# hir0shim/singleSpMV

Hardware: NVIDIA B200
Metric: SpMV GFLOP/s (higher is better)
Workload: dtype f64

## Files before the change

singlespmv_b200/csrc/chunk_stream.cu:

```cuda
#include <algorithm>
#include <climits>
#include <cstdlib>
#include <cstring>
#include <map>

#include "chunk_stream.cuh"

namespace b2 {

template <typename VT, typename XT, typename AT, int MAXL, int TH, bool ACC, bool DICT>
__global__ void __launch_bounds__(TH)
chunk_stream_kernel(const int *__restrict__ ptr, const int *__restrict__ idx, const int *__restrict__ meta,
                    const VT *__restrict__ val, const XT *__restrict__ x, XT *__restrict__ y, int rowBegin, int rowEnd,
                    int chunk0, int nChunks, int capI, int capV, int S, int acc_mode)
{
    constexpr int MI = CS_META_INTS(TH);
    extern __shared__ __align__(128) unsigned char cs_smem[];
    __shared__ __align__(8) uint64_t bar[CS_MAXSTAGES];
    __shared__ int sbaseI[CS_MAXSTAGES], sbaseV[CS_MAXSTAGES];
    int *sidx = reinterpret_cast<int *>(cs_smem);
    VT *sval = reinterpret_cast<VT *>(cs_smem + (size_t)S * capI * sizeof(int));
    const int tid = threadIdx.x;
    const uint64_t pol_stream = policy_evict_first(), pol_x = policy_evict_last();

    auto issue = [&](int s, long long g, int b, int e) {
        const int *srcI = idx + b;
        const VT *srcV = val + b;
        const int misI = (int)((reinterpret_cast<uintptr_t>(srcI) & 15) / sizeof(int));
        const int misV = (int)((reinterpret_cast<uintptr_t>(srcV) & 15) / sizeof(VT));
        const int n = e - b;
        const uint32_t bytesI = DICT ? (uint32_t)(MI * sizeof(int)) : n ? (uint32_t)(((n + misI) * (int)sizeof(int) + 15) & ~15) : 0u;
        const uint32_t bytesV = n ? (uint32_t)(((n + misV) * (int)sizeof(VT) + 15) & ~15) : 0u;
        sbaseI[s] = b - misI;
        sbaseV[s] = b - misV;
        mbar_expect_tx(&bar[s], bytesI + bytesV);
        if (DICT) tma_load_1d(sidx + (size_t)s * capI, meta + g * MI, bytesI, &bar[s], pol_stream);
        if (n) {
            if (!DICT) tma_load_1d(sidx + (size_t)s * capI, srcI - misI, bytesI, &bar[s], pol_stream);
            tma_load_1d(sval + (size_t)s * capV, srcV - misV, bytesV, &bar[s], pol_stream);
        }
    };
    auto lo_of = [&](long long g) { return (int)min((long long)rowEnd, max((long long)rowBegin, g * TH)); };

    if (tid == 0)
        for (int s = 0; s < S; s++) mbar_init(&bar[s], 1);
    __syncthreads();
    if (tid == 0) {
        for (int s = 0; s < S; s++) {
            const long long c = (long long)blockIdx.x + (long long)s * gridDim.x;
            if (c < nChunks) issue(s, chunk0 + c, ptr[lo_of(chunk0 + c)], ptr[lo_of(chunk0 + c + 1)]);
        }
    }
    long long g = (long long)chunk0 + blockIdx.x;
    int r = (int)min(g * TH + tid, (long long)0x7fffffff);
    bool valid = r >= rowBegin && r < rowEnd;
    int p = 0, q = 0;
    if (!DICT && valid) {
        p = ptr[r];
        q = ptr[r + 1];
    }
    int k = 0;
    for (long long c = blockIdx.x; c < nChunks; c += gridDim.x, k++) {
        const int s = k % S;
        const long long cIssue = c + (long long)S * gridDim.x, cNext = c + gridDim.x;
        int nb = 0, ne = 0, pn = 0, qn = 0;
        if (tid == 0 && cIssue < nChunks) {
            nb = ptr[lo_of(chunk0 + cIssue)];
            ne = ptr[lo_of(chunk0 + cIssue + 1)];
        }
        const long long rnl = (chunk0 + cNext) * TH + tid;
        const int rn = (int)min(rnl, (long long)0x7fffffff);
        const bool validn = cNext < nChunks && rn >= rowBegin && rn < rowEnd;
        if (!DICT && validn) {
            pn = ptr[rn];
            qn = ptr[rn + 1];
        }
        const AT y0 = (ACC && valid) ? (AT)y[r] : (AT)0;
        mbar_wait(&bar[s], (uint32_t)(k / S) & 1u);
        AT acc = (ACC && acc_mode == CS_CONTINUE) ? y0 : (AT)0;
        XT xs[MAXL];
        int len, vo;
        if (DICT) {
            const int *rec = sidx + (size_t)s * capI;
            const uint32_t mrow = reinterpret_cast<const uint16_t *>(rec + CS_DICT + TH / 32)[tid];
            const int lane = tid & 31, cnt = __popc(mrow);
            int inc = cnt;
#pragma unroll
            for (int o = 1; o < 32; o <<= 1) {
                const int t = __shfl_up_sync(0xffffffffu, inc, o);
                if (lane >= o) inc += t;
            }
            vo = s * capV + (rec[CS_DICT + (tid >> 5)] + inc - cnt - sbaseV[s]);
            uint32_t m = valid ? mrow : 0u;
            len = __popc(m);
#pragma unroll
            for (int j = 0; j < MAXL; j++)
                if (j < len) {
                    xs[j] = ld_x(x + (r + rec[__ffs(m) - 1]), pol_x);
                    m &= m - 1;
                }
        } else {
            const int io = s * capI + (p - sbaseI[s]);
            vo = s * capV + (p - sbaseV[s]);
            len = q - p;
#pragma unroll
            for (int j = 0; j < MAXL; j++)
                if (j < len) xs[j] = ld_x(x + sidx[io + j], pol_x);
        }
#pragma unroll
        for (int j = 0; j < MAXL; j++)
            if (j < len) acc = Arith<AT>::add(acc, Arith<AT>::mul((AT)sval[vo + j], (AT)xs[j]));
        if (valid) y[r] = (XT)((ACC && acc_mode == CS_ADD) ? Arith<AT>::add(y0, acc) : acc);
        __syncthreads();
        if (tid == 0 && cIssue < nChunks) issue(s, chunk0 + cIssue, nb, ne);
        r = rn; p = pn; q = qn; valid = validn;
    }
}

__global__ void chunk_cap_kernel(const int *__restrict__ ptr, int nRow, int th, int nChunks, int *__restrict__ out)
{
    const int c = blockIdx.x * blockDim.x + threadIdx.x;
    int n = 0;
    if (c < nChunks) n = ptr[(int)min((long long)nRow, ((long long)c + 1) * th)] - ptr[(long long)c * th];
#pragma unroll
    for (int o = 16; o > 0; o >>= 1) n = max(n, __shfl_xor_sync(0xffffffffu, n, o));
    if ((threadIdx.x & 31) == 0 && n > 0) atomicMax(out, n);
}

template <int TH>
__global__ void __launch_bounds__(TH)
chunk_dict_kernel(const int *__restrict__ ptr, const int *__restrict__ idx, int nRow, int *__restrict__ meta,
                  int *__restrict__ overflow)
{
    __shared__ int red[2][TH / 32];
    __shared__ int dict[CS_DICT];
    const int tid = threadIdx.x, lane = tid & 31, w = tid >> 5;
    const long long r = (long long)blockIdx.x * TH + tid;
    int b = 0, n = 0;
    if (r < nRow) {
        b = ptr[r];
        n = ptr[r + 1] - b;
    }
    int off[CS_MAXLEN];
#pragma unroll
    for (int j = 0; j < CS_MAXLEN; j++) off[j] = j < n ? idx[b + j] - (int)r : INT_MAX;
    int nd = 0;
    for (int cur = INT_MIN;;) {
        int mn = INT_MAX;
#pragma unroll
        for (int j = 0; j < CS_MAXLEN; j++)
            if (off[j] > cur) mn = min(mn, off[j]);
        mn = __reduce_min_sync(0xffffffffu, mn);
        if (lane == 0) red[nd & 1][w] = mn;
        __syncthreads();
        mn = INT_MAX;
#pragma unroll
        for (int i = 0; i < TH / 32; i++) mn = min(mn, red[nd & 1][i]);
        if (mn == INT_MAX) break;
        if (nd == CS_DICT) {
            if (tid == 0) *overflow = 1;
            return;
        }
        if (tid == 0) dict[nd] = mn;
        cur = mn;
        nd++;
    }
    uint32_t m = 0;
    int last = -1;
    bool bad = false;
#pragma unroll
    for (int j = 0; j < CS_MAXLEN; j++)
        if (j < n) {
            int k = 0;
            for (int i = 0; i < nd; i++) k += dict[i] < off[j];
            bad |= k <= last;
            last = k;
            m |= 1u << k;
        }
    if (bad) *overflow = 1;
    int *rec = meta + (size_t)blockIdx.x * CS_META_INTS(TH);
    if (tid < CS_DICT) rec[tid] = tid < nd ? dict[tid] : 0;
    if (lane == 0) rec[CS_DICT + w] = ptr[min(r, (long long)nRow)];
    reinterpret_cast<uint16_t *>(rec + CS_DICT + TH / 32)[tid] = (uint16_t)m;
}

int ChunkStream::build(const int *ptr_d, const int *idx_d, const void *val_d, bool val_is_f32, int nRow_, int nnz,
                       int maxLen_, cudaStream_t s)
{
    ptr = ptr_d; idx = idx_d; val = val_d; f32 = val_is_f32; nRow = nRow_; maxLen = maxLen_;
    feed = CS_FEED_IDX;
    meta.release();
    static const int env_max = getenv("B200SPMV_TMA_MAXLEN") ? atoi(getenv("B200SPMV_TMA_MAXLEN")) : CS_MAXLEN;
    const int env_th = getenv("B200SPMV_TMA_R") ? atoi(getenv("B200SPMV_TMA_R")) : 0;
    ok = nnz > 0 && nRow > 0 && maxLen > 0 && maxLen <= std::min(env_max, CS_MAXLEN);
    if (!ok) return B200SPMV_OK;
    th = env_th == 512 ? 512 : 256;
    const int nChunks = ceil_div(nRow, th);
    const char *env_feed = getenv("B200SPMV_CS_FEED");
    const bool want_dict = !(env_feed && !strcmp(env_feed, "idx"));
    DevBuf<int> m;
    B2_TRY(m.alloc(2));
    B2_CUDA(cudaMemsetAsync(m.p, 0, 2 * sizeof(int), s));
    chunk_cap_kernel<<<ceil_div(nChunks, 256), 256, 0, s>>>(ptr, nRow, th, nChunks, m.p);
    B2_KERNEL_CHECK();
    const size_t metaInts = (size_t)nChunks * CS_META_INTS(th);
    if (want_dict) {
        B2_TRY(meta.alloc(metaInts + CS_SLACK));
        B2_CUDA(cudaMemsetAsync(meta.p + metaInts, 0, CS_SLACK * sizeof(int), s));
        if (th == 512) chunk_dict_kernel<512><<<nChunks, 512, 0, s>>>(ptr, idx, nRow, meta.p, m.p + 1);
        else chunk_dict_kernel<256><<<nChunks, 256, 0, s>>>(ptr, idx, nRow, meta.p, m.p + 1);
        B2_KERNEL_CHECK();
    }
    int h[2] = {0, 0};
    B2_CUDA(cudaMemcpyAsync(h, m.p, sizeof h, cudaMemcpyDeviceToHost, s));
    B2_CUDA(cudaStreamSynchronize(s));
    cap = h[0];
    if (want_dict && !h[1]) feed = CS_FEED_DICT;
    else meta.release();
    const size_t stage = (size_t)(cap + 16) * (f32 ? 4 : 8) + (feed == CS_FEED_DICT ? CS_META_INTS(th) * 4 : (size_t)(cap + 16) * 4);
    if (2 * stage > 200 * 1024) ok = false;
    return B200SPMV_OK;
}

template <typename VT, typename XT, typename AT, int MAXL, int TH, bool ACC, bool DICT>
static int cs_launch(const ChunkStream &c, const XT *x, XT *y, int rb, int re, int acc, cudaStream_t s)
{
    constexpr int VA = 16 / (int)sizeof(VT);
    static const int env_s = getenv("B200SPMV_TMA_S") ? atoi(getenv("B200SPMV_TMA_S")) : 0;
    static const int env_b = getenv("B200SPMV_TMA_CTAS") ? atoi(getenv("B200SPMV_TMA_CTAS")) : 0;
    const int S = (env_s >= 1 && env_s <= CS_MAXSTAGES) ? env_s : 2;
    const int capI = DICT ? CS_META_INTS(TH) : (c.cap + 8) & ~3, capV = (c.cap + 2 * VA) & ~(VA - 1);
    const size_t smem = (size_t)S * ((size_t)capI * 4 + (size_t)capV * sizeof(VT));
    auto kern = chunk_stream_kernel<VT, XT, AT, MAXL, TH, ACC, DICT>;
    static int sms = 0;
    static std::map<std::pair<int, size_t>, int> per_sm;
    int dev = 0;
    B2_CUDA(cudaGetDevice(&dev));
    if (!sms) B2_CUDA(cudaDeviceGetAttribute(&sms, cudaDevAttrMultiProcessorCount, dev));
    const auto key = std::make_pair(dev, smem);
    auto it = per_sm.find(key);
    if (it == per_sm.end()) {
        B2_CUDA(cudaFuncSetAttribute(kern, cudaFuncAttributeMaxDynamicSharedMemorySize, (int)std::max<size_t>(smem, 200 * 1024)));
        int n = 0;
        B2_CUDA(cudaOccupancyMaxActiveBlocksPerMultiprocessor(&n, kern, TH, smem));
        if (n < 1) { set_error("row-chunk stream: %zu bytes of shared memory do not fit", smem); return B200SPMV_ERR_UNSUPPORTED; }
        it = per_sm.emplace(key, n).first;
    }
    const int perSm = env_b > 0 ? std::min(it->second, env_b) : it->second;
    const int chunk0 = rb / TH, nChunks = ceil_div(re, TH) - chunk0;
    const int grid = std::min(nChunks, sms * perSm);
    kern<<<grid, TH, smem, s>>>(c.ptr, c.idx, c.meta.p, static_cast<const VT *>(c.val), x, y, rb, re, chunk0, nChunks, capI, capV, S, acc);
    B2_KERNEL_CHECK();
    return B200SPMV_OK;
}

template <typename VT, typename XT, typename AT, int MAXL, int TH, bool ACC>
static int cs_feed(const ChunkStream &c, const XT *x, XT *y, int rb, int re, int acc, cudaStream_t s)
{
    if (c.feed == CS_FEED_DICT) return cs_launch<VT, XT, AT, MAXL, TH, ACC, true>(c, x, y, rb, re, acc, s);
    return cs_launch<VT, XT, AT, MAXL, TH, ACC, false>(c, x, y, rb, re, acc, s);
}

template <typename VT, typename XT, typename AT>
static int cs_dispatch(const ChunkStream &c, const XT *x, XT *y, int rb, int re, int acc, cudaStream_t s)
{
#define CS_GO(MAXL)                                                                                       \
    do {                                                                                                  \
        if (c.th == 512 && acc) return cs_feed<VT, XT, AT, MAXL, 512, true>(c, x, y, rb, re, acc, s);   \
        if (c.th == 512) return cs_feed<VT, XT, AT, MAXL, 512, false>(c, x, y, rb, re, acc, s);         \
        if (acc) return cs_feed<VT, XT, AT, MAXL, 256, true>(c, x, y, rb, re, acc, s);                  \
        return cs_feed<VT, XT, AT, MAXL, 256, false>(c, x, y, rb, re, acc, s);                          \
    } while (0)
    if (c.maxLen <= 8) CS_GO(8);
    else CS_GO(16);
#undef CS_GO
}

int ChunkStream::run(const double *x, double *y, int rb, int re, int acc, cudaStream_t s) const
{
    if (rb < 0 || re > nRow || rb > re) { set_error("multiply_rows: bad row range [%d,%d) for %d rows", rb, re, nRow); return B200SPMV_ERR_INVALID; }
    if (rb == re) return B200SPMV_OK;
    if (f32) return cs_dispatch<float, double, double>(*this, x, y, rb, re, acc, s);
    return cs_dispatch<double, double, double>(*this, x, y, rb, re, acc, s);
}

int ChunkStream::run_f32(const float *x, float *y, int rb, int re, int acc, bool acc64, cudaStream_t s) const
{
    if (rb < 0 || re > nRow || rb > re) { set_error("multiply_rows: bad row range [%d,%d) for %d rows", rb, re, nRow); return B200SPMV_ERR_INVALID; }
    if (!f32) { set_error("row-chunk stream: fp32 vectors need fp32 value storage"); return B200SPMV_ERR_STATE; }
    if (rb == re) return B200SPMV_OK;
    if (acc64) return cs_dispatch<float, float, double>(*this, x, y, rb, re, acc, s);
    return cs_dispatch<float, float, float>(*this, x, y, rb, re, acc, s);
}

}
```

singlespmv_b200/csrc/chunk_stream.cuh:

```cuda
#pragma once
#include "common.cuh"

namespace b2 {

constexpr int CS_MAXLEN = 16;
constexpr int CS_SLACK = 8;
constexpr int CS_MAXSTAGES = 4;

constexpr int CS_DICT = 16;
__host__ __device__ constexpr int CS_META_INTS(int th) { return CS_DICT + th / 32 + th / 2; }
enum { CS_FEED_IDX = 0, CS_FEED_DICT = 1 };

struct ChunkStream {
    const int *ptr = nullptr, *idx = nullptr;
    const void *val = nullptr;
    bool f32 = false, ok = false;
    int nRow = 0, maxLen = 0, th = 0, cap = 0;
    int feed = CS_FEED_IDX;
    DevBuf<int> meta;

    int build(const int *ptr_d, const int *idx_d, const void *val_d, bool val_is_f32, int nRow_, int nnz, int maxLen_,
              cudaStream_t s);
    int run(const double *x, double *y, int rb, int re, int acc, cudaStream_t s) const;
    int run_f32(const float *x, float *y, int rb, int re, int acc, bool acc64, cudaStream_t s) const;
};

}
```

singlespmv_b200/csrc/crs.cu:

```cuda
#include <algorithm>
#include <cstdlib>
#include <cstring>

#include "chunk_stream.cuh"
#include "entry_stream.cuh"
#include "tile_stream.cuh"

namespace b2 {

__global__ void crs_to_f32_kernel(const double *__restrict__ in, int n, float *__restrict__ out)
{
    const int i = blockIdx.x * blockDim.x + threadIdx.x;
    if (i < n) out[i] = __double2float_rn(in[i]);
}
__global__ void crs_to_f64_kernel(const float *__restrict__ in, int n, double *__restrict__ out)
{
    const int i = blockIdx.x * blockDim.x + threadIdx.x;
    if (i < n) out[i] = (double)in[i];
}

constexpr int RBS_MAXLEN = 16;
constexpr int RBS_WARPS = 8;
constexpr int RBS_ITERS = 8;

// ... 81 lines not shown
    EntryStream es;
    bool use_es = false;
    int path_opt;
    int prec;
    explicit CrsFormat(const b200spmv_options &o) : f32(o.value_f32 != 0 || o.precision != 0), path_opt(o.crs_path), prec(o.precision) {}

    int convert(const CooView &A, cudaStream_t s) override
    {
        nRow = A.nRow; nCol = A.nCol; nnz = A.nnz;
        B2_TRY(validate_sorted_coo(A, s));
        B2_TRY(ptr.alloc((size_t)nRow + 1));
        B2_TRY(idx.alloc((size_t)nnz + CS_SLACK));
        B2_TRY(build_row_ptr(A.row, nnz, nRow, ptr.p, s));
        B2_CUDA(cudaMemcpyAsync(idx.p, A.col, sizeof(int) * (size_t)nnz, cudaMemcpyDeviceToDevice, s));
        if (f32) {
            val.release();
            B2_TRY(val32.alloc((size_t)nnz + CS_SLACK));
            if (nnz) crs_to_f32_kernel<<<ceil_div(nnz, 256), 256, 0, s>>>(A.val, nnz, val32.p);
            B2_KERNEL_CHECK();
            B2_TRY(ts.build(ptr.p, idx.p, val32.p, true, nRow, nnz, s));
        } else {
            B2_TRY(val.alloc((size_t)nnz + CS_SLACK));
            B2_CUDA(cudaMemcpyAsync(val.p, A.val, sizeof(double) * (size_t)nnz, cudaMemcpyDeviceToDevice, s));
            B2_TRY(ts.build(ptr.p, idx.p, val.p, false, nRow, nnz, s));
        }
        B2_TRY(max_row_length(ptr.p, nRow, &maxLen, s));
        B2_TRY(cs.build(ptr.p, idx.p, f32 ? (const void *)val32.p : (const void *)val.p, f32, nRow, nnz, maxLen, s));
        use_rbs = path_opt == 2 && !prec && rowblock_applies(maxLen, nnz);
        int band = 0;
        if (path_opt == 0 || path_opt == 4) B2_TRY(max_band(A.row, A.col, nnz, A.rowOffset, &band, s));
        short_rows = path_opt != 1 && path_opt != 4 && (use_rbs || (cs.ok && !gathers_need_l2(band)));
        static const char *force = getenv("B200SPMV_CRS_PATH");
        use_es = false;
        const bool force_es = force && !strcmp(force, "es") && path_opt == 0;
        if (!short_rows && !f32 && !prec && (path_opt == 4 || force_es || (path_opt == 0 && gathers_need_l2(band))) && !(force && !strcmp(force, "tile"))) {
            B2_TRY(es.build(ptr.p, idx.p, val.p, nRow, nnz, gathers_need_l2(band), s));
            use_es = es.ok;
        }
        B2_CUDA(cudaStreamSynchronize(s));
        return B200SPMV_OK;
    }

    int multiply(const double *x, double *y, cudaStream_t s) override { return multiply_rows(0, nRow, x, y, s); }
    int multiply_f32(const float *x, float *y, cudaStream_t s) override
    {
        if (!prec) { set_error("multiply_f32: the handle was created with precision = 0 (fp64 vectors)"); return B200SPMV_ERR_STATE; }
        if (short_rows && !use_rbs) return cs.run_f32(x, y, 0, nRow, CS_OVERWRITE, prec == 2, s);
        return ts.run_rows_f32(x, y, CS_OVERWRITE, 0, nRow, prec == 2, s);
    }

    int multiply_rows(int rb, int re, const double *x, double *y, cudaStream_t s) override
    {
        if (prec) { set_error("multiply: the handle was created with precision = %d, use b200spmv_multiply_f32", prec); return B200SPMV_ERR_STATE; }
        if (!short_rows && use_es) return es.run_rows(x, y, rb, re, s);
        if (!short_rows) return ts.run_rows(x, y, CS_OVERWRITE, rb, re, s);
        if (rb < 0 || re > nRow || rb > re) { set_error("multiply_rows: bad row range [%d,%d)", rb, re); return B200SPMV_ERR_INVALID; }
        if (rb == re) return B200SPMV_OK;
        if (use_rbs) return rowblock_spmv(ptr.p, idx.p, f32 ? (const void *)val32.p : (const void *)val.p, f32, maxLen, rb, re, x, y, s);
        return cs.run(x, y, rb, re, CS_OVERWRITE, s);
    }
    bool has_rows() const override { return !prec; }
    int prepare_rows(int rb, int re) override { return short_rows ? B200SPMV_OK : use_es ? es.prepare(rb, re) : ts.prepare(rb, re); }
    int col_extent(int rb, int re, int *cmin, int *cmax) override
    {
        if (rb < 0 || re > nRow || rb > re) { set_error("col_extent: bad row range [%d,%d)", rb, re); return B200SPMV_ERR_INVALID; }
        int pb = 0, pe = 0;
        B2_CUDA(cudaMemcpy(&pb, ptr.p + rb, sizeof(int), cudaMemcpyDeviceToHost));
        B2_CUDA(cudaMemcpy(&pe, ptr.p + re, sizeof(int), cudaMemcpyDeviceToHost));
        if (pe <= pb) { *cmin = 0; *cmax = -1; return B200SPMV_OK; }
        return minmax_i32(idx.p, pb, pe, cmin, cmax);
    }

    bool scalar(const std::string &n, long long *out) override
    {
        if (n == "alg_bytes") {
            *out = (f32 ? 8LL : 12LL) * nnz + 4LL * (nRow + 1) + (prec ? 4LL : 8LL) * ((long long)nCol + nRow);
            return true;
        }
        if (n == "launches") { *out = short_rows ? 1 : use_es ? (es.nTiles > 1 ? 2 : 1) + (es.nEmpty ? 1 : 0) : (ts.nTiles > 1 ? 2 : 1); return true; }
        if (n == "crs_kernel") { *out = short_rows ? 1 : use_es ? (es.tma ? 2 : 3) : 0; return true; }
        if (n == "maxLength") { *out = maxLen; return true; }
        if (n == "short_row_path") { *out = short_rows ? 1 : 0; return true; }
        if (n == "chunk_feed") { *out = short_rows && !use_rbs ? cs.feed : CS_FEED_IDX; return true; }
        if (n == "nTiles") { *out = ts.nTiles; return true; }
        if (n == "value_f32") { *out = f32 ? 1 : 0; return true; }
        if (n == "precision") { *out = prec; return true; }
        return false;
    }

    long long array(const std::string &n, void *dst, long long cap) override
    {
        if (n == "ptr") return export_device(ptr.p, ptr.bytes(), dst, cap);
        if (n == "idx") return export_device(idx.p, sizeof(int) * (size_t)nnz, dst, cap);
        if (n == "val") {
            if (!f32) return export_device(val.p, sizeof(double) * (size_t)nnz, dst, cap);
            if (!dst) return (long long)(sizeof(double) * (size_t)nnz);
            DevBuf<double> w;
            if (w.alloc((size_t)nnz)) return B200SPMV_ERR_NOMEM;
            if (nnz) crs_to_f64_kernel<<<ceil_div(nnz, 256), 256>>>(val32.p, nnz, w.p);
            return export_device(w.p, w.bytes(), dst, cap);
        }
        return -1000;
    }
};

Format *make_crs(const b200spmv_options &o) { return new CrsFormat(o); }

}
```

singlespmv_b200/csrc/ss.cu:

```cuda
#include <algorithm>
#include <cstdlib>
#include <cstring>
#include <cub/cub.cuh>

#include "chunk_stream.cuh"
#include "colblocks.cuh"
#include "tile_stream.cuh"

namespace b2 {

__global__ void ss_slab_kernel(const int *__restrict__ row, const int *__restrict__ col, const double *__restrict__ val,
                               long long nnz, long long slots, int padRow, int *__restrict__ row2d,
                               int *__restrict__ col2d, double *__restrict__ val2d)
{
    const long long p = (long long)blockIdx.x * blockDim.x + threadIdx.x;
    if (p >= slots) return;
    const bool real = p < nnz;
    row2d[p] = real ? row[p] : padRow;
    col2d[p] = real ? col[p] : 0;
    val2d[p] = real ? val[p] : 0.0;
}

__global__ void chain_mixed_kernel(const int *__restrict__ row2d, long long slots, int W, int *__restrict__ mixed)
{
// ... 219 lines not shown
    {
        nRow = A.nRow; nCol = A.nCol; nnz = A.nnz;
        B2_TRY(validate_sorted_coo(A, s));
        H = nnz / W + (nnz % W != 0);
        const long long slots = (long long)H * W;
        B2_TRY(row_ptr.alloc((size_t)nRow + 1));
        B2_TRY(row2d.alloc((size_t)slots));
        B2_TRY(col2d.alloc((size_t)slots + CS_SLACK));
        B2_TRY(val2d.alloc((size_t)slots + CS_SLACK));
        B2_TRY(seg_index.alloc((size_t)H));
        B2_TRY(build_row_ptr(A.row, nnz, nRow, row_ptr.p, s));
        if (slots) {
            ss_slab_kernel<<<ceil_div(slots, 256), 256, 0, s>>>(A.row, A.col, A.val, nnz, slots, nRow, row2d.p, col2d.p, val2d.p);
            B2_KERNEL_CHECK();
        }
        B2_TRY(build_chain(row2d.p, H, W, seg_index.p, &nStep, counts, segs, s));
        B2_TRY(ts.build(row_ptr.p, col2d.p, val2d.p, false, nRow, nnz, s));
        B2_TRY(max_row_length(row_ptr.p, nRow, &maxLen, s));
        B2_TRY(cs.build(row_ptr.p, col2d.p, val2d.p, false, nRow, nnz, maxLen, s));
        use_rbs = path_opt == 2 && rowblock_applies(maxLen, nnz);
        int band = 0;
        if (path_opt == 0 && cs.ok) B2_TRY(max_band(A.row, A.col, nnz, A.rowOffset, &band, s));
        short_rows = path_opt != 1 && (use_rbs || (cs.ok && !gathers_need_l2(band)));
        cb.reset();
        if (!faithful) B2_TRY(make_col_block_engine(A, row_ptr.p, cbs_want, s, &cb));
        if (faithful) B2_TRY(val_buf.alloc((size_t)slots));
        B2_CUDA(cudaStreamSynchronize(s));
        return B200SPMV_OK;
    }

    int multiply(const double *x, double *y, cudaStream_t s) override
    {
        if (!faithful) return multiply_rows(0, nRow, x, y, s);
        if (nRow == 0) return B200SPMV_OK;
        const long long slots = (long long)H * W;
        B2_TRY(prof.mark(0, s));
        if (slots) {
            ss_mul_kernel<<<ceil_div(slots, 256), 256, 0, s>>>(col2d.p, val2d.p, x, slots, val_buf.p);
            B2_KERNEL_CHECK();
        }
        B2_TRY(prof.mark(1, s));
        B2_TRY(faithful_fold(segs, counts, W, val_buf.p, s));
        ss_gather_kernel<<<ceil_div(nRow, 256), 256, 0, s>>>(row_ptr.p, val_buf.p, nRow, W, 0, y);
        B2_KERNEL_CHECK();
        B2_TRY(prof.mark(2, s));
        return prof.finish();
    }

    bool has_rows() const override { return !faithful && !(cb != nullptr); }
    int prepare_rows(int rb, int re) override
    {
        if (faithful) return B200SPMV_OK;
        if (cb != nullptr) return cb->prepare(rb, re);
        return short_rows ? B200SPMV_OK : ts.prepare(rb, re);
    }
    int col_extent(int rb, int re, int *cmin, int *cmax) override
    {
        if (rb < 0 || re > nRow || rb > re) { set_error("col_extent: bad row range [%d,%d)", rb, re); return B200SPMV_ERR_INVALID; }
        int pb = 0, pe = 0;
        B2_CUDA(cudaMemcpy(&pb, row_ptr.p + rb, sizeof(int), cudaMemcpyDeviceToHost));
        B2_CUDA(cudaMemcpy(&pe, row_ptr.p + re, sizeof(int), cudaMemcpyDeviceToHost));
        if (pe <= pb) { *cmin = 0; *cmax = -1; return B200SPMV_OK; }
        return minmax_i32(col2d.p, pb, pe, cmin, cmax);
    }
    int multiply_rows(int rb, int re, const double *x, double *y, cudaStream_t s) override
    {
        if (faithful) return Format::multiply_rows(rb, re, x, y, s);
        if ((cb != nullptr)) return cb->run(x, y, rb, re, s);
        if (short_rows) {
            if (rb < 0 || re > nRow || rb > re) { set_error("multiply_rows: bad row range [%d,%d)", rb, re); return B200SPMV_ERR_INVALID; }
            if (use_rbs) return rowblock_spmv(row_ptr.p, col2d.p, val2d.p, false, maxLen, rb, re, x, y, s);
            return cs.run(x, y, rb, re, CS_OVERWRITE, s);
        }
        return ts.run_rows(x, y, CS_OVERWRITE, rb, re, s);
    }

    bool scalar(const std::string &n, long long *out) override
    {
        if (prof.scalar(n, out)) return true;
        if (n == "col_blocks") { *out = (cb != nullptr) ? cb->n_blocks() : 0; return true; }
        if (n == "col_block_engine") { *out = (cb == nullptr) ? 0 : (cb->name()[0] == 'e' ? 1 : 2); return true; }
        if (n == "short_row_path") { *out = short_rows ? 1 : 0; return true; }
        if (n == "chunk_feed") { *out = !faithful && cb == nullptr && short_rows && !use_rbs ? cs.feed : CS_FEED_IDX; return true; }
        if (n == "H") { *out = H; return true; }
        if (n == "nStep") { *out = nStep; return true; }
        if (n == "W") { *out = W; return true; }
        if (n == "alg_bytes") {
            *out = 12LL * nnz + 4LL * (nRow + 1) + 8LL * nCol + 8LL * nRow;
            return true;
        }
        if (n == "launches") {
            if (!faithful) { *out = (cb != nullptr) ? cb->n_blocks() : short_rows ? 1 : (ts.nTiles > 1 ? 2 : 1); return true; }
            int l = 2;
            for (int c : counts) l += c > 0;
            *out = l;
            return true;
        }
        return false;
    }

    long long array(const std::string &n, void *dst, long long cap) override
    {
        if (n == "row_ptr") return export_device(row_ptr.p, row_ptr.bytes(), dst, cap);
        if (n == "row_idx") return export_device(row2d.p, row2d.bytes(), dst, cap);
        if (n == "col_idx") return export_device(col2d.p, sizeof(int) * (size_t)H * W, dst, cap);
        if (n == "val") return export_device(val2d.p, sizeof(double) * (size_t)H * W, dst, cap);
        if (n == "segment_index") return export_device(seg_index.p, seg_index.bytes(), dst, cap);
        if (n == "sum_segs") return export_device(segs.p, segs.bytes(), dst, cap);
        if (n == "sum_segs_count") return export_host(counts.data(), counts.size() * sizeof(int), dst, cap);
        return -1000;
    }
};

Format *make_ss(const b200spmv_options &o) { return new SsFormat(o); }

constexpr int CSS_HIST = 1024;
__global__ void css_block_key_kernel(const int *__restrict__ col, int nnz, int B, int nBlock, int *__restrict__ key,
                                     int *__restrict__ id, int *__restrict__ blockNnz)
{
    __shared__ int hist[CSS_HIST];
    const bool local = nBlock <= CSS_HIST;
    if (local)
        for (int k = threadIdx.x; k < nBlock; k += blockDim.x) hist[k] = 0;
    __syncthreads();
    for (int i = blockIdx.x * blockDim.x + threadIdx.x; i < nnz; i += gridDim.x * blockDim.x) {
        const int b = col[i] / B;
        key[i] = b;
        id[i] = i;
        atomicAdd(local ? &hist[b] : &blockNnz[b], 1);
    }
    __syncthreads();
    if (local)
        for (int k = threadIdx.x; k < nBlock; k += blockDim.x)
            if (hist[k]) atomicAdd(&blockNnz[k], hist[k]);
}
__global__ void css_scatter_kernel(const int *__restrict__ row, const int *__restrict__ col, const double *__restrict__ val,
                                   const int *__restrict__ key_sorted, const int *__restrict__ id_sorted, int nnz,
                                   const long long *__restrict__ slabBase, const int *__restrict__ blockStart,
                                   int *__restrict__ row2d, int *__restrict__ col2d, double *__restrict__ val2d)
{
    const int k = blockIdx.x * blockDim.x + threadIdx.x;
    if (k >= nnz) return;
    const int b = key_sorted[k], i = id_sorted[k];
    const long long p = slabBase[b] + (k - blockStart[b]);
    row2d[p] = row[i];
    col2d[p] = col[i];
    val2d[p] = val[i];
}

__global__ void colblock_spread_kernel(const int *__restrict__ ptr, const int *__restrict__ col, int nRow, int B,
                                       unsigned long long *__restrict__ stats)
{
    const int r = blockIdx.x * blockDim.x + threadIdx.x;
    int touched = 0, nonEmpty = 0;
    if (r < nRow) {
        int last = -1;
        for (int j = ptr[r]; j < ptr[r + 1]; j++) {
            const int b = col[j] / B;
            touched += b != last;
            last = b;
        }
        nonEmpty = touched > 0;
    }
#pragma unroll
    for (int o = 16; o > 0; o >>= 1) {
        touched += __shfl_xor_sync(0xffffffffu, touched, o);
// ... 141 lines not shown
        if (!faithful) {
            if (ellb) return ellb->run(x, y, 0, nRow, s);
            for (int b = 0; b < nBlock; b++) B2_TRY(blocks[(size_t)b]->run(x, y, 0, nRow, gather_bound, b > 0 ? CS_ADD : CS_OVERWRITE, s));
            return B200SPMV_OK;
        }
        const long long slots = (long long)totalH * W;
        B2_TRY(prof.mark(0, s));
        if (slots) {
            ss_mul_kernel<<<ceil_div(slots, 256), 256, 0, s>>>(col2d.p, val2d.p, x, slots, val_buf.p);
            B2_KERNEL_CHECK();
        }
        B2_TRY(prof.mark(1, s));
        B2_CUDA(cudaMemsetAsync(y, 0, sizeof(double) * (size_t)nRow, s));
        for (int b = 0; b < nBlock; b++) {
            CssBlock &k = *blocks[(size_t)b];
            B2_TRY(faithful_fold(k.segs, k.counts, W, val_buf.p + k.base, s));
            ss_gather_kernel<<<ceil_div(nRow, 256), 256, 0, s>>>(row_ptr.p + (size_t)b * ((size_t)nRow + 1), val_buf.p + k.base,
                                                                nRow, W, 1, y);
            B2_KERNEL_CHECK();
        }
        B2_TRY(prof.mark(2, s));
        return prof.finish();
    }

    bool has_rows() const override { return !faithful; }
    int prepare_rows(int rb, int re) override
    {
        if (faithful || ellb || (rb == 0 && re == nRow)) return B200SPMV_OK;
        for (auto &k : blocks) if (!k->cs.ok || gather_bound) B2_TRY(k->ts.prepare(rb, re));
        return B200SPMV_OK;
    }
    int multiply_rows(int rb, int re, const double *x, double *y, cudaStream_t s) override
    {
        if (faithful) return Format::multiply_rows(rb, re, x, y, s);
        if (rb < 0 || re > nRow || rb > re) { set_error("multiply_rows: bad row range [%d,%d)", rb, re); return B200SPMV_ERR_INVALID; }
        if (rb == re) return B200SPMV_OK;
        if (nBlock == 0) {
            B2_CUDA(cudaMemsetAsync(y + rb, 0, sizeof(double) * (size_t)(re - rb), s));
            return B200SPMV_OK;
        }
        if (ellb) return ellb->run(x, y, rb, re, s);
        for (int b = 0; b < nBlock; b++) B2_TRY(blocks[(size_t)b]->run(x, y, rb, re, gather_bound, b > 0 ? CS_ADD : CS_OVERWRITE, s));
        return B200SPMV_OK;
    }
    int multiply_continue(int rb, int re, const double *x, double *y, cudaStream_t s)
    {
        bool first = true;
        for (auto &k : blocks) {
            if (k->cnt == 0 && !first) continue;
            if (k->cnt == 0) { B2_CUDA(cudaMemsetAsync(y + rb, 0, sizeof(double) * (size_t)(re - rb), s)); first = false; continue; }
            B2_TRY(k->run(x, y, rb, re, gather_bound, first ? CS_OVERWRITE : CS_CONTINUE, s));
            first = false;
        }
        return B200SPMV_OK;
    }

    int n_x_slices() const override { return faithful || nBlock < 1 ? 1 : nBlock; }
    void x_slice(int i, long long *c0, long long *c1) const override
    {
        if (faithful || nBlock < 1) { *c0 = 0; *c1 = nCol; return; }
        *c0 = (long long)i * B;
        *c1 = std::min<long long>(nCol, *c0 + B);
    }
    int multiply_rows_slice(int i, int rb, int re, const double *x, double *y, cudaStream_t s) override
    {
        if (faithful || nBlock < 1) return multiply_rows(rb, re, x, y, s);
        if (ellb) return ellb->run_block(i, x, y, rb, re, s);
        return blocks[(size_t)i]->run(x, y, rb, re, gather_bound, i > 0 ? CS_ADD : CS_OVERWRITE, s);
    }

    bool scalar(const std::string &n, long long *out) override
    {
        if (prof.scalar(n, out)) return true;
        if (n == "B") { *out = B; return true; }
        if (n == "col_block_engine") { *out = ellb ? 1 : (gather_bound ? 2 : 0); return true; }
        if (n == "nBlock") { *out = nBlock; return true; }
        if (n == "chunk_feed") {
            bool any = false, all = true;
            if (!faithful && !ellb && !gather_bound)
                for (auto &k : blocks) if (k->cs.ok) { any = true; all = all && k->cs.feed == CS_FEED_DICT; }
            *out = any && all ? CS_FEED_DICT : CS_FEED_IDX;
            return true;
        }
        if (n == "totalH") { *out = totalH; return true; }
        if (n == "W") { *out = W; return true; }
        if (n == "alg_bytes") {
            *out = 12LL * nnz + 4LL * nBlock * ((long long)nRow + 1) + 8LL * nCol + 8LL * nRow;
            return true;
        }
        if (n == "launches") {
            long long l = 0;
            if (!faithful && ellb) l = ellb->n_blocks();
            else if (!faithful) for (auto &k : blocks) l += k->cs.ok ? 1 : (k->ts.nTiles > 1 ? 2 : 1);
            else { l = 2; for (auto &k : blocks) { l += 1; for (int c : k->counts) l += c > 0; } }
            *out = l;
            return true;
        }
        return false;
    }

    long long array(const std::string &n, void *dst, long long cap) override
    {
        if (n == "row_ptr") return export_device(row_ptr.p, row_ptr.bytes(), dst, cap);
        if (n == "row_idx") return export_device(row2d.p, row2d.bytes(), dst, cap);
        if (n == "col_idx") return export_device(col2d.p, sizeof(int) * (size_t)totalH * W, dst, cap);
        if (n == "val") return export_device(val2d.p, sizeof(double) * (size_t)totalH * W, dst, cap);
        if (n == "segment_index") return export_device(seg_index.p, seg_index.bytes(), dst, cap);
        std::vector<int> h;
        if (n == "H") { for (auto &k : blocks) h.push_back(k->H); return export_host(h.data(), h.size() * sizeof(int), dst, cap); }
        if (n == "nStep") { for (auto &k : blocks) h.push_back(k->nStep); return export_host(h.data(), h.size() * sizeof(int), dst, cap); }
        if (n == "sum_segs_count") {
            for (auto &k : blocks) h.insert(h.end(), k->counts.begin(), k->counts.end());
            return export_host(h.data(), h.size() * sizeof(int), dst, cap);
        }
        if (n == "sum_segs") {
            size_t total = 0;
            for (auto &k : blocks) total += k->segs.n;
            if (!dst) return (long long)(total * sizeof(int));
            if (cap < (long long)(total * sizeof(int))) { set_error("get_array: destination too small"); return B200SPMV_ERR_INVALID; }
            size_t at = 0;
            for (auto &k : blocks) {
                if (k->segs.n && cudaMemcpy((int *)dst + at, k->segs.p, k->segs.bytes(), cudaMemcpyDeviceToHost) != cudaSuccess) {
                    set_error("get_array: cudaMemcpy D2H failed");
                    return B200SPMV_ERR_CUDA;
                }
                at += k->segs.n;
            }
            return (long long)(total * sizeof(int));
        }
        return -1000;
    }
};

Format *make_css(const b200spmv_options &o) { return new CssFormat(o); }

struct CrsColBlocks : ColBlockEngine {
    CssFormat css;
    explicit CrsColBlocks(const b200spmv_options &o) : css(o) { css.lean = true; css.input_checked = true; }
    int run(const double *x, double *y, int rb, int re, cudaStream_t s) override { return css.multiply_continue(rb, re, x, y, s); }
    int prepare(int rb, int re) override { return css.prepare_rows(rb, re); }
    int n_blocks() const override { return css.nBlock; }
    const char *name() const override { return "crs"; }
};
int make_col_block_engine(const CooView &A, const int *row_ptr, int want, cudaStream_t s, std::unique_ptr<ColBlockEngine> *out)
{
    out->reset();
    static const char *env_n = getenv("B200SPMV_COL_BLOCKS");
    if (env_n) want = atoi(env_n) == 0 ? -1 : atoi(env_n);
    if (want < 0 || A.nnz == 0 || A.nRow == 0 || A.nCol == 0) return B200SPMV_OK;
    int nb = want;
    if (want == 0) {
        if ((long long)A.nCol * 8 <= 64LL << 20) return B200SPMV_OK;
        nb = (int)(((long long)A.nCol * 8 + COLBLOCK_SLICE_BYTES - 1) / COLBLOCK_SLICE_BYTES);
        if (nb > COLBLOCK_MAX) nb = COLBLOCK_MAX;
        const int B = (A.nCol + nb - 1) / nb;
        DevBuf<unsigned long long> stats;
        B2_TRY(stats.alloc(2));
        B2_CUDA(cudaMemsetAsync(stats.p, 0, stats.bytes(), s));
        colblock_spread_kernel<<<ceil_div(A.nRow, 256), 256, 0, s>>>(row_ptr, A.col, A.nRow, B, stats.p);
        B2_KERNEL_CHECK();
        unsigned long long st[2] = {0, 0};
        B2_CUDA(cudaMemcpyAsync(st, stats.p, sizeof st, cudaMemcpyDeviceToHost, s));
        B2_CUDA(cudaStreamSynchronize(s));
        if ((double)st[0] < 1.5 * (double)st[1]) return B200SPMV_OK;
    }
    const char *env_e = getenv("B200SPMV_COL_BLOCK_ENGINE");
// ... 16 lines not shown
```

Before: 1145.

## Compress chunk values into 4-bit codes with per-chunk value tables

Adds a value-dictionary feed to the chunked TMA SpMV. When a chunk has at most 16 distinct values, each nonzero's value is stored as a 4-bit code in a packed array, and a 16-entry table is appended to the chunk's metadata record. The streaming kernel TMA-loads the codes instead of the full values and decodes them through the table in shared memory, cutting streamed value bytes. It also adds a min-blocks launch bound for short-row, non-accumulating variants. The cost is extra preprocessing and decode work, and the path only applies to matrices with few distinct values per chunk.

```diff
diff --git a/singlespmv_b200/csrc/chunk_stream.cu b/singlespmv_b200/csrc/chunk_stream.cu
--- a/singlespmv_b200/csrc/chunk_stream.cu
+++ b/singlespmv_b200/csrc/chunk_stream.cu
@@ -8,36 +8,54 @@
 
 namespace b2 {
 
-template <typename VT, typename XT, typename AT, int MAXL, int TH, bool ACC, bool DICT>
-__global__ void __launch_bounds__(TH)
-chunk_stream_kernel(const int *__restrict__ ptr, const int *__restrict__ idx, const int *__restrict__ meta,
-                    const VT *__restrict__ val, const XT *__restrict__ x, XT *__restrict__ y, int rowBegin, int rowEnd,
-                    int chunk0, int nChunks, int capI, int capV, int S, int acc_mode)
-{
-    constexpr int MI = CS_META_INTS(TH);
+enum { CSK_IDX = 0, CSK_OFFSETS = 1, CSK_VALUES = 2 };
+
+#define CS_MIN_CTAS(MAXL, TH, ACC, FEED) (((FEED) == CSK_VALUES && (MAXL) <= 8 && !(ACC)) ? 2048 / (TH) : 0)
+
+template <typename VT, typename XT, typename AT, int MAXL, int TH, bool ACC, int FEED>
+__global__ void __launch_bounds__(TH, CS_MIN_CTAS(MAXL, TH, ACC, FEED))
+chunk_stream_kernel(const int *__restrict__ ptr, const int *__restrict__ idx, const int *__restrict__ meta, int recInts,
+                    const VT *__restrict__ val, const uint8_t *__restrict__ codes, const XT *__restrict__ x,
+                    XT *__restrict__ y, int rowBegin, int rowEnd, int chunk0, int nChunks, int capI, int capV, int S,
+                    int acc_mode)
+{
+    constexpr bool DICT = FEED != CSK_IDX, VALS = FEED == CSK_VALUES;
+    constexpr int MI = CS_META_INTS(TH), RI = MI + (VALS ? CS_TAB_INTS(sizeof(VT)) : 0);
     extern __shared__ __align__(128) unsigned char cs_smem[];
     __shared__ __align__(8) uint64_t bar[CS_MAXSTAGES];
     __shared__ int sbaseI[CS_MAXSTAGES], sbaseV[CS_MAXSTAGES];
     int *sidx = reinterpret_cast<int *>(cs_smem);
-    VT *sval = reinterpret_cast<VT *>(cs_smem + (size_t)S * capI * sizeof(int));
+    unsigned char *sv = cs_smem + (size_t)S * capI * sizeof(int);
+    const VT *sval = reinterpret_cast<const VT *>(sv);
     const int tid = threadIdx.x;
-    const uint64_t pol_stream = policy_evict_first(), pol_x = policy_evict_last();
+    const uint64_t pol_x = policy_evict_last();
 
     auto issue = [&](int s, long long g, int b, int e) {
+        const uint64_t pol_stream = policy_evict_first();
+        const int n = e - b;
         const int *srcI = idx + b;
-        const VT *srcV = val + b;
         const int misI = (int)((reinterpret_cast<uintptr_t>(srcI) & 15) / sizeof(int));
-        const int misV = (int)((reinterpret_cast<uintptr_t>(srcV) & 15) / sizeof(VT));
-        const int n = e - b;
-        const uint32_t bytesI = DICT ? (uint32_t)(MI * sizeof(int)) : n ? (uint32_t)(((n + misI) * (int)sizeof(int) + 15) & ~15) : 0u;
-        const uint32_t bytesV = n ? (uint32_t)(((n + misV) * (int)sizeof(VT) + 15) & ~15) : 0u;
+        const uint32_t bytesI = DICT ? (uint32_t)(RI * sizeof(int)) : n ? (uint32_t)(((n + misI) * (int)sizeof(int) + 15) & ~15) : 0u;
+        const void *srcV;
+        uint32_t bytesV;
+        if (VALS) {
+            const uint8_t *c = codes + (b >> 1);
+            const int mis = (int)(reinterpret_cast<uintptr_t>(c) & 15);
+            srcV = c - mis;
+            bytesV = n ? (uint32_t)((((e + 1) >> 1) - (b >> 1) + mis + 15) & ~15) : 0u;
+            sbaseV[s] = 2 * ((b >> 1) - mis);
+        } else {
+            const int misV = (int)((reinterpret_cast<uintptr_t>(val + b) & 15) / sizeof(VT));
+            srcV = val + b - misV;
+            bytesV = n ? (uint32_t)(((n + misV) * (int)sizeof(VT) + 15) & ~15) : 0u;
+            sbaseV[s] = b - misV;
+        }
         sbaseI[s] = b - misI;
-        sbaseV[s] = b - misV;
         mbar_expect_tx(&bar[s], bytesI + bytesV);
-        if (DICT) tma_load_1d(sidx + (size_t)s * capI, meta + g * MI, bytesI, &bar[s], pol_stream);
+        if (DICT) tma_load_1d(sidx + (size_t)s * capI, meta + g * recInts, bytesI, &bar[s], pol_stream);
         if (n) {
             if (!DICT) tma_load_1d(sidx + (size_t)s * capI, srcI - misI, bytesI, &bar[s], pol_stream);
-            tma_load_1d(sval + (size_t)s * capV, srcV - misV, bytesV, &bar[s], pol_stream);
+            tma_load_1d(sv + (size_t)s * capV * (VALS ? 1 : sizeof(VT)), srcV, bytesV, &bar[s], pol_stream);
         }
     };
     auto lo_of = [&](long long g) { return (int)min((long long)rowEnd, max((long long)rowBegin, g * TH)); };
@@ -60,15 +78,15 @@
         q = ptr[r + 1];
     }
     int k = 0;
-    for (long long c = blockIdx.x; c < nChunks; c += gridDim.x, k++) {
+    for (int c = blockIdx.x; c < nChunks; c += gridDim.x, k++) {
         const int s = k % S;
-        const long long cIssue = c + (long long)S * gridDim.x, cNext = c + gridDim.x;
+        const int cIssue = c + S * (int)gridDim.x, cNext = c + (int)gridDim.x;
         int nb = 0, ne = 0, pn = 0, qn = 0;
         if (tid == 0 && cIssue < nChunks) {
             nb = ptr[lo_of(chunk0 + cIssue)];
             ne = ptr[lo_of(chunk0 + cIssue + 1)];
         }
-        const long long rnl = (chunk0 + cNext) * TH + tid;
+        const long long rnl = ((long long)chunk0 + cNext) * TH + tid;
         const int rn = (int)min(rnl, (long long)0x7fffffff);
         const bool validn = cNext < nChunks && rn >= rowBegin && rn < rowEnd;
         if (!DICT && validn) {
@@ -79,9 +97,10 @@
         mbar_wait(&bar[s], (uint32_t)(k / S) & 1u);
         AT acc = (ACC && acc_mode == CS_CONTINUE) ? y0 : (AT)0;
         XT xs[MAXL];
-        int len, vo;
+        int len, vo = 0;
+        uint32_t c0 = 0, c1 = 0;
+        const int *rec = sidx + (size_t)s * capI;
         if (DICT) {
-            const int *rec = sidx + (size_t)s * capI;
             const uint32_t mrow = reinterpret_cast<const uint16_t *>(rec + CS_DICT + TH / 32)[tid];
             const int lane = tid & 31, cnt = __popc(mrow);
             int inc = cnt;
@@ -90,9 +109,19 @@
                 const int t = __shfl_up_sync(0xffffffffu, inc, o);
                 if (lane >= o) inc += t;
             }
-            vo = s * capV + (rec[CS_DICT + (tid >> 5)] + inc - cnt - sbaseV[s]);
+            const int first = rec[CS_DICT + (tid >> 5)] + inc - cnt;
             uint32_t m = valid ? mrow : 0u;
             len = __popc(m);
+            if (VALS) {
+                if (len) {
+                    const int nib = first - sbaseV[s];
+                    const uint32_t *w = reinterpret_cast<const uint32_t *>(sv + (size_t)s * capV) + (nib >> 3);
+                    c0 = __funnelshift_r(w[0], w[1], (nib & 7) * 4);
+                    if (MAXL > 8) c1 = __funnelshift_r(w[1], w[2], (nib & 7) * 4);
+                }
+            } else {
+                vo = s * capV + (first - sbaseV[s]);
+            }
 #pragma unroll
             for (int j = 0; j < MAXL; j++)
                 if (j < len) {
@@ -107,9 +136,13 @@
             for (int j = 0; j < MAXL; j++)
                 if (j < len) xs[j] = ld_x(x + sidx[io + j], pol_x);
         }
+        const VT *tab = reinterpret_cast<const VT *>(rec + MI);
 #pragma unroll
         for (int j = 0; j < MAXL; j++)
-            if (j < len) acc = Arith<AT>::add(acc, Arith<AT>::mul((AT)sval[vo + j], (AT)xs[j]));
+            if (j < len) {
+                const VT v = VALS ? tab[((j < 8 ? c0 : c1) >> (4 * (j & 7))) & 15u] : sval[vo + j];
+                acc = Arith<AT>::add(acc, Arith<AT>::mul((AT)v, (AT)xs[j]));
+            }
         if (valid) y[r] = (XT)((ACC && acc_mode == CS_ADD) ? Arith<AT>::add(y0, acc) : acc);
         __syncthreads();
         if (tid == 0 && cIssue < nChunks) issue(s, chunk0 + cIssue, nb, ne);
@@ -127,13 +160,16 @@
     if ((threadIdx.x & 31) == 0 && n > 0) atomicMax(out, n);
 }
 
-template <int TH>
+template <int TH, typename UT>
 __global__ void __launch_bounds__(TH)
-chunk_dict_kernel(const int *__restrict__ ptr, const int *__restrict__ idx, int nRow, int *__restrict__ meta,
-                  int *__restrict__ overflow)
+chunk_dict_kernel(const int *__restrict__ ptr, const int *__restrict__ idx, const UT *__restrict__ vbits, int nRow,
+                  int recInts, int *__restrict__ meta, uint32_t *__restrict__ codes, int *__restrict__ out)
 {
     __shared__ int red[2][TH / 32];
     __shared__ int dict[CS_DICT];
+    __shared__ UT vred[2][TH / 32];
+    __shared__ UT vtab[CS_VTAB];
+    __shared__ uint32_t scode[CS_MAXLEN * TH / 8 + 2];
     const int tid = threadIdx.x, lane = tid & 31, w = tid >> 5;
     const long long r = (long long)blockIdx.x * TH + tid;
     int b = 0, n = 0;
@@ -158,7 +194,7 @@
         for (int i = 0; i < TH / 32; i++) mn = min(mn, red[nd & 1][i]);
         if (mn == INT_MAX) break;
         if (nd == CS_DICT) {
-            if (tid == 0) *overflow = 1;
+            if (tid == 0) out[0] = 1;
             return;
         }
         if (tid == 0) dict[nd] = mn;
@@ -177,11 +213,58 @@
             last = k;
             m |= 1u << k;
         }
-    if (bad) *overflow = 1;
-    int *rec = meta + (size_t)blockIdx.x * CS_META_INTS(TH);
+    if (bad) out[0] = 1;
+    int *rec = meta + (size_t)blockIdx.x * recInts;
     if (tid < CS_DICT) rec[tid] = tid < nd ? dict[tid] : 0;
     if (lane == 0) rec[CS_DICT + w] = ptr[min(r, (long long)nRow)];
     reinterpret_cast<uint16_t *>(rec + CS_DICT + TH / 32)[tid] = (uint16_t)m;
+    if (!codes) return;
+
+    for (int i = tid; i < CS_MAXLEN * TH / 8 + 2; i += TH) scode[i] = 0;
+    UT v[CS_MAXLEN];
+#pragma unroll
+    for (int j = 0; j < CS_MAXLEN; j++) v[j] = j < n ? vbits[b + j] : (UT)0;
+    int nv = 0;
+    for (UT cur = 0;;) {
+        UT mn = ~(UT)0;
+        bool any = false;
+#pragma unroll
+        for (int j = 0; j < CS_MAXLEN; j++)
+            if (j < n && (nv == 0 || v[j] > cur)) {
+                mn = min(mn, v[j]);
+                any = true;
+            }
+#pragma unroll
+        for (int o = 16; o > 0; o >>= 1) mn = min(mn, (UT)__shfl_xor_sync(0xffffffffu, mn, o));
+        if (lane == 0) vred[nv & 1][w] = mn;
+        if (!__syncthreads_or(any)) break;
+        mn = ~(UT)0;
+#pragma unroll
+        for (int i = 0; i < TH / 32; i++) mn = min(mn, vred[nv & 1][i]);
+        if (nv == CS_VTAB) {
+            if (tid == 0) out[1] = 1;
+            return;
+        }
+        if (tid == 0) vtab[nv] = mn;
+        cur = mn;
+        nv++;
+    }
+    const int e0 = ptr[(long long)blockIdx.x * TH] & ~7, e1 = ptr[min((long long)blockIdx.x * TH + TH, (long long)nRow)];
+#pragma unroll
+    for (int j = 0; j < CS_MAXLEN; j++)
+        if (j < n) {
+            uint32_t k = 0;
+            for (int i = 0; i < nv; i++) k += vtab[i] < v[j];
+            atomicOr(&scode[(b + j - e0) >> 3], k << (4 * ((b + j) & 7)));
+        }
+    UT *tab = reinterpret_cast<UT *>(rec + CS_META_INTS(TH));
+    if (tid < CS_VTAB) tab[tid] = tid < nv ? vtab[tid] : (UT)0;
+    __syncthreads();
+    const int nw = (e1 - e0 + 7) >> 3;
+    for (int i = tid; i < nw; i += TH) {
+        if (i == 0 || i == nw - 1) atomicOr(&codes[(e0 >> 3) + i], scode[i]);
+        else codes[(e0 >> 3) + i] = scode[i];
+    }
 }
 
 int ChunkStream::build(const int *ptr_d, const int *idx_d, const void *val_d, bool val_is_f32, int nRow_, int nnz,
@@ -189,7 +272,9 @@
 {
     ptr = ptr_d; idx = idx_d; val = val_d; f32 = val_is_f32; nRow = nRow_; maxLen = maxLen_;
     feed = CS_FEED_IDX;
+    vfeed = CS_VALUES_RUN;
     meta.release();
+    codes.release();
     static const int env_max = getenv("B200SPMV_TMA_MAXLEN") ? atoi(getenv("B200SPMV_TMA_MAXLEN")) : CS_MAXLEN;
     const int env_th = getenv("B200SPMV_TMA_R") ? atoi(getenv("B200SPMV_TMA_R")) : 0;
     ok = nnz > 0 && nRow > 0 && maxLen > 0 && maxLen <= std::min(env_max, CS_MAXLEN);
@@ -198,40 +283,61 @@
     const int nChunks = ceil_div(nRow, th);
     const char *env_feed = getenv("B200SPMV_CS_FEED");
     const bool want_dict = !(env_feed && !strcmp(env_feed, "idx"));
+    const bool want_vals = want_dict && !(env_feed && !strcmp(env_feed, "offsets"));
     DevBuf<int> m;
-    B2_TRY(m.alloc(2));
-    B2_CUDA(cudaMemsetAsync(m.p, 0, 2 * sizeof(int), s));
+    B2_TRY(m.alloc(3));
+    B2_CUDA(cudaMemsetAsync(m.p, 0, 3 * sizeof(int), s));
     chunk_cap_kernel<<<ceil_div(nChunks, 256), 256, 0, s>>>(ptr, nRow, th, nChunks, m.p);
     B2_KERNEL_CHECK();
-    const size_t metaInts = (size_t)nChunks * CS_META_INTS(th);
+    recInts = CS_META_INTS(th) + (want_vals ? CS_TAB_INTS(f32 ? 4 : 8) : 0);
+    const size_t metaInts = (size_t)nChunks * recInts;
     if (want_dict) {
         B2_TRY(meta.alloc(metaInts + CS_SLACK));
         B2_CUDA(cudaMemsetAsync(meta.p + metaInts, 0, CS_SLACK * sizeof(int), s));
-        if (th == 512) chunk_dict_kernel<512><<<nChunks, 512, 0, s>>>(ptr, idx, nRow, meta.p, m.p + 1);
-        else chunk_dict_kernel<256><<<nChunks, 256, 0, s>>>(ptr, idx, nRow, meta.p, m.p + 1);
+        uint32_t *cp = nullptr;
+        if (want_vals) {
+            const size_t words = (size_t)(nnz + 7) / 8 + CS_SLACK;
+            B2_TRY(codes.alloc(words));
+            B2_CUDA(cudaMemsetAsync(codes.p, 0, words * sizeof(uint32_t), s));
+            cp = codes.p;
+        }
+#define CS_DICT_GO(TH, UT) chunk_dict_kernel<TH, UT><<<nChunks, TH, 0, s>>>(ptr, idx, static_cast<const UT *>(val), nRow, recInts, meta.p, cp, m.p + 1)
+        if (th == 512 && f32) CS_DICT_GO(512, uint32_t);
+        else if (th == 512) CS_DICT_GO(512, uint64_t);
+        else if (f32) CS_DICT_GO(256, uint32_t);
+        else CS_DICT_GO(256, uint64_t);
+#undef CS_DICT_GO
         B2_KERNEL_CHECK();
     }
-    int h[2] = {0, 0};
+    int h[3] = {0, 0, 0};
     B2_CUDA(cudaMemcpyAsync(h, m.p, sizeof h, cudaMemcpyDeviceToHost, s));
     B2_CUDA(cudaStreamSynchronize(s));
     cap = h[0];
-    if (want_dict && !h[1]) feed = CS_FEED_DICT;
-    else meta.release();
-    const size_t stage = (size_t)(cap + 16) * (f32 ? 4 : 8) + (feed == CS_FEED_DICT ? CS_META_INTS(th) * 4 : (size_t)(cap + 16) * 4);
+    if (want_dict && !h[1]) {
+        feed = CS_FEED_DICT;
+        if (want_vals && !h[2]) vfeed = CS_VALUES_CODES;
+        else codes.release();
+    } else {
+        meta.release();
+        codes.release();
+    }
+    const size_t stage = (vfeed == CS_VALUES_CODES ? (size_t)cap / 2 + 48 : (size_t)(cap + 16) * (f32 ? 4 : 8)) +
+                         (feed == CS_FEED_DICT ? (size_t)recInts * 4 : (size_t)(cap + 16) * 4);
     if (2 * stage > 200 * 1024) ok = false;
     return B200SPMV_OK;
 }
 
-template <typename VT, typename XT, typename AT, int MAXL, int TH, bool ACC, bool DICT>
+template <typename VT, typename XT, typename AT, int MAXL, int TH, bool ACC, int FEED>
 static int cs_launch(const ChunkStream &c, const XT *x, XT *y, int rb, int re, int acc, cudaStream_t s)
 {
     constexpr int VA = 16 / (int)sizeof(VT);
     static const int env_s = getenv("B200SPMV_TMA_S") ? atoi(getenv("B200SPMV_TMA_S")) : 0;
     static const int env_b = getenv("B200SPMV_TMA_CTAS") ? atoi(getenv("B200SPMV_TMA_CTAS")) : 0;
     const int S = (env_s >= 1 && env_s <= CS_MAXSTAGES) ? env_s : 2;
-    const int capI = DICT ? CS_META_INTS(TH) : (c.cap + 8) & ~3, capV = (c.cap + 2 * VA) & ~(VA - 1);
-    const size_t smem = (size_t)S * ((size_t)capI * 4 + (size_t)capV * sizeof(VT));
-    auto kern = chunk_stream_kernel<VT, XT, AT, MAXL, TH, ACC, DICT>;
+    const int capI = FEED != CSK_IDX ? c.recInts : (c.cap + 8) & ~3;
+    const int capV = FEED == CSK_VALUES ? ((c.cap + 1) / 2 + 47) & ~15 : (c.cap + 2 * VA) & ~(VA - 1);
+    const size_t smem = (size_t)S * ((size_t)capI * 4 + (size_t)capV * (FEED == CSK_VALUES ? 1 : sizeof(VT)));
+    auto kern = chunk_stream_kernel<VT, XT, AT, MAXL, TH, ACC, FEED>;
     static int sms = 0;
     static std::map<std::pair<int, size_t>, int> per_sm;
     int dev = 0;
@@ -249,7 +355,8 @@
     const int perSm = env_b > 0 ? std::min(it->second, env_b) : it->second;
     const int chunk0 = rb / TH, nChunks = ceil_div(re, TH) - chunk0;
     const int grid = std::min(nChunks, sms * perSm);
-    kern<<<grid, TH, smem, s>>>(c.ptr, c.idx, c.meta.p, static_cast<const VT *>(c.val), x, y, rb, re, chunk0, nChunks, capI, capV, S, acc);
+    kern<<<grid, TH, smem, s>>>(c.ptr, c.idx, c.meta.p, c.recInts, static_cast<const VT *>(c.val),
+                                reinterpret_cast<const uint8_t *>(c.codes.p), x, y, rb, re, chunk0, nChunks, capI, capV, S, acc);
     B2_KERNEL_CHECK();
     return B200SPMV_OK;
 }
@@ -257,8 +364,9 @@
 template <typename VT, typename XT, typename AT, int MAXL, int TH, bool ACC>
 static int cs_feed(const ChunkStream &c, const XT *x, XT *y, int rb, int re, int acc, cudaStream_t s)
 {
-    if (c.feed == CS_FEED_DICT) return cs_launch<VT, XT, AT, MAXL, TH, ACC, true>(c, x, y, rb, re, acc, s);
-    return cs_launch<VT, XT, AT, MAXL, TH, ACC, false>(c, x, y, rb, re, acc, s);
+    if (c.feed == CS_FEED_DICT && c.vfeed == CS_VALUES_CODES) return cs_launch<VT, XT, AT, MAXL, TH, ACC, CSK_VALUES>(c, x, y, rb, re, acc, s);
+    if (c.feed == CS_FEED_DICT) return cs_launch<VT, XT, AT, MAXL, TH, ACC, CSK_OFFSETS>(c, x, y, rb, re, acc, s);
+    return cs_launch<VT, XT, AT, MAXL, TH, ACC, CSK_IDX>(c, x, y, rb, re, acc, s);
 }
 
 template <typename VT, typename XT, typename AT>
diff --git a/singlespmv_b200/csrc/chunk_stream.cuh b/singlespmv_b200/csrc/chunk_stream.cuh
--- a/singlespmv_b200/csrc/chunk_stream.cuh
+++ b/singlespmv_b200/csrc/chunk_stream.cuh
@@ -10,6 +10,9 @@
 constexpr int CS_DICT = 16;
 __host__ __device__ constexpr int CS_META_INTS(int th) { return CS_DICT + th / 32 + th / 2; }
 enum { CS_FEED_IDX = 0, CS_FEED_DICT = 1 };
+constexpr int CS_VTAB = 16;
+__host__ __device__ constexpr int CS_TAB_INTS(int vt_size) { return CS_VTAB * vt_size / 4; }
+enum { CS_VALUES_RUN = 0, CS_VALUES_CODES = 1 };
 
 struct ChunkStream {
     const int *ptr = nullptr, *idx = nullptr;
@@ -17,7 +20,10 @@
     bool f32 = false, ok = false;
     int nRow = 0, maxLen = 0, th = 0, cap = 0;
     int feed = CS_FEED_IDX;
+    int vfeed = CS_VALUES_RUN;
+    int recInts = 0;
     DevBuf<int> meta;
+    DevBuf<uint32_t> codes;
 
     int build(const int *ptr_d, const int *idx_d, const void *val_d, bool val_is_f32, int nRow_, int nnz, int maxLen_,
               cudaStream_t s);
diff --git a/singlespmv_b200/csrc/crs.cu b/singlespmv_b200/csrc/crs.cu
--- a/singlespmv_b200/csrc/crs.cu
+++ b/singlespmv_b200/csrc/crs.cu
@@ -187,6 +187,7 @@
         if (n == "maxLength") { *out = maxLen; return true; }
         if (n == "short_row_path") { *out = short_rows ? 1 : 0; return true; }
         if (n == "chunk_feed") { *out = short_rows && !use_rbs ? cs.feed : CS_FEED_IDX; return true; }
+        if (n == "value_feed") { *out = short_rows && !use_rbs ? cs.vfeed : CS_VALUES_RUN; return true; }
         if (n == "nTiles") { *out = ts.nTiles; return true; }
         if (n == "value_f32") { *out = f32 ? 1 : 0; return true; }
         if (n == "precision") { *out = prec; return true; }
diff --git a/singlespmv_b200/csrc/ss.cu b/singlespmv_b200/csrc/ss.cu
--- a/singlespmv_b200/csrc/ss.cu
+++ b/singlespmv_b200/csrc/ss.cu
@@ -325,6 +325,7 @@
         if (n == "col_block_engine") { *out = (cb == nullptr) ? 0 : (cb->name()[0] == 'e' ? 1 : 2); return true; }
         if (n == "short_row_path") { *out = short_rows ? 1 : 0; return true; }
         if (n == "chunk_feed") { *out = !faithful && cb == nullptr && short_rows && !use_rbs ? cs.feed : CS_FEED_IDX; return true; }
+        if (n == "value_feed") { *out = !faithful && cb == nullptr && short_rows && !use_rbs ? cs.vfeed : CS_VALUES_RUN; return true; }
         if (n == "H") { *out = H; return true; }
         if (n == "nStep") { *out = nStep; return true; }
         if (n == "W") { *out = W; return true; }
@@ -632,6 +633,13 @@
             *out = any && all ? CS_FEED_DICT : CS_FEED_IDX;
             return true;
         }
+        if (n == "value_feed") {
+            bool any = false, all = true;
+            if (!faithful && !ellb && !gather_bound)
+                for (auto &k : blocks) if (k->cs.ok) { any = true; all = all && k->cs.vfeed == CS_VALUES_CODES; }
+            *out = any && all ? CS_VALUES_CODES : CS_VALUES_RUN;
+            return true;
+        }
         if (n == "totalH") { *out = totalH; return true; }
         if (n == "W") { *out = W; return true; }
         if (n == "alg_bytes") {
```

Result: faster. 1215, median of 6 (+6.1%).
